# antgroup/ant-ray

Measured on NVIDIA H100. Metric: resnet50_ddp_train_images_per_sec, higher is better.
Workload: dtype bf16

## Files before the change

ant-ray_b200/csrc/inst_norm.cu:

```cuda
#include <algorithm>
#include <initializer_list>
#include <type_traits>

#include "norm_act.cuh"
#include "norm_infer.cuh"
#include "norm_kernels.cuh"
#include "norm_launch.h"
#include "norm_res.cuh"

namespace b200c {
namespace bn {

static int ceil_div(int a, int b) { return (a + b - 1) / b; }

static int last_pow2(unsigned n) {
  n |= (n >> 1);
  n |= (n >> 2);
  n |= (n >> 4);
  n |= (n >> 8);
  n |= (n >> 16);
  return std::max<int>(1, n - (n >> 1));
}

static void reduce_config(int reduction, int stride, dim3* block, dim3* grid) {
  int block_x = std::min(last_pow2(stride), kTileW);
  int block_y = std::min(last_pow2(ceil_div(reduction, kElemsPerThread)), kMaxBlock / block_x);
  if (block_x * block_y != kMaxBlock) block_x = std::min(last_pow2(stride), kMaxBlock / block_y);
  int grid_y = std::min(ceil_div(reduction, block_y * kElemsPerThread), kMaxHBlock);
  *block = dim3(block_x, block_y, 1);
  *grid = dim3(ceil_div(stride, block_x), grid_y < 8 ? 1 : grid_y, 1);
}

static_assert(kEwVec % kStatsVec == 0, "vec_ok covers the statistics kernel's vector width");
static bool vec_ok(int stride, const void* const* ptrs, int n) {
  if (stride % kEwVec) return false;
  for (int i = 0; i < n; i++)
    if (reinterpret_cast<uintptr_t>(ptrs[i]) % 16) return false;
  return true;
}

constexpr size_t kBlockSmem = 48 * 1024;
constexpr size_t kStatsStaticSmem = 3 * kMaxBlock * 4 + 16;
constexpr size_t kBwdStaticSmem = 2 * kMaxBlock * 4 + 16;

static size_t stats_ring_bytes(dim3 block) {
  return (size_t)kStatsStages * kParallelLoads * block.x * block.y * sizeof(BVec<kStatsVec>);
}
static_assert(kStatsStaticSmem + (size_t)kStatsStages * kParallelLoads * (kMaxBlock / kStatsVec) * sizeof(BVec<kStatsVec>) <= kBlockSmem,
              "the statistics ring fits every block");

static_assert(kBwdStaticSmem + (size_t)kBwdStagesWide * 5 * kParallelLoads * (kMaxBlock / kBwdVec) * sizeof(BVec<kBwdVec>) <= kBlockSmem &&
                  kBwdStaticSmem + (size_t)kBwdStages * 2 * kParallelLoads * (kMaxBlock / kBwdVec) * sizeof(BVec<kBwdVec>) <= kBlockSmem,
              "the backward ring fits every block: 2 stages of up to 5 operands, 3 of 2");
struct BwdReduceLaunch {
  dim3 block, grid;
  int vec;
  size_t smem;
};
static BwdReduceLaunch bwd_reduce_launch(int m, int c, GradSrc src, bool dy2, bool dual, const void* const* ptrs, int n) {
  BwdReduceLaunch l;
  reduce_config(m, c, &l.block, &l.grid);
  l.vec = 1;
  l.smem = 0;
  if (src == kGradPool || !vec_ok(c, ptrs, n)) return l;
  const int ops = bwd_ring_operands(src == kGradY, dy2, dual);
  const size_t ring = (size_t)bwd_ring_stages(ops) * ops * kParallelLoads * (l.block.x / kBwdVec) * l.block.y * sizeof(BVec<kBwdVec>);
  l.block.x /= kBwdVec;
  l.vec = kBwdVec;
  l.smem = ring;
  return l;
}

static void ew_config(int reduction, int stride, int vec, dim3* block, dim3* grid) {
  const int groups = stride / vec;
  const int bx = std::min(groups, kEwThreads);
  const int by = kEwThreads / bx;
  const int gx = ceil_div(groups, bx);
  const int gy = std::max(1, std::min(ceil_div(reduction, by), 4096 / gx));
  *block = dim3(bx, by, 1);
  *grid = dim3(gx, gy, 1);
}

constexpr int kSemaphores = kMaxChannels / kTileW;
constexpr size_t kSemaphoreBytes = (size_t)kSemaphores * 4;

size_t scratch_bytes(int stride) {
  return kSemaphoreBytes + (size_t)3 * stride * kMaxHBlock * 4 + (size_t)2 * stride * 4;
}

struct Scratch {
  int* semaphores;
  float* staging;
  float* sums;
};
static Scratch carve(void* scratch, int stride) {
  char* p = static_cast<char*>(scratch);
  Scratch s;
  s.semaphores = reinterpret_cast<int*>(p);
  s.staging = reinterpret_cast<float*>(p + kSemaphoreBytes);
  s.sums = s.staging + (size_t)3 * stride * kMaxHBlock;
  return s;
}

template <int... Cs, typename F>
static auto with_const(int key, F&& f) {
  std::common_type_t<decltype(f(std::integral_constant<int, Cs>{}))...> kernel = nullptr;
  ((key == Cs ? void(kernel = f(std::integral_constant<int, Cs>{})) : void()), ...);
  return kernel;
}

using StatsKernel = void (*)(const bf16*, StatsOut, volatile float*, int*, int, int);
using SyncStatsKernel = void (*)(const bf16*, float*, float, volatile float*, int*, int, int);
using StatsDualKernel = void (*)(const bf16*, const bf16*, StatsOut, StatsOut, volatile float*, volatile float*, int*, int, int);
using TransformKernel = void (*)(const bf16*, const bf16*, bf16*, uint8_t*, const float*, const float*, const float*, const float*,
                                 const float*, const float*, const float*, const float*, int, int);
using PoolFwdKernel = void (*)(const bf16*, bf16*, uint8_t*, const float*, const float*, const float*, const float*, PoolDims, int, int);
using BwdReduceKernel = void (*)(const bf16*, const bf16*, const bf16*, const bf16*, const uint8_t*, bf16*, const float*, const float*,
                                 float*, float*, float*, float*, volatile float*, int*, PoolDims, const bf16*, const float*, const float*,
                                 float*, float*, float*, int, int, int);
using BwdElemtKernel = void (*)(const bf16*, const bf16*, const bf16*, const uint8_t*, const bf16*, bf16*, const float*, const float*,
                                const float*, const float*, const float*, const float*, float, const bf16*, bf16*, const float*,
                                const float*, const float*, const float*, int, int);

static StatsKernel stats_kernel(int vec) {
  return with_const<1, kStatsVec>(vec, [](auto v) -> StatsKernel { return k_bn_stats<decltype(v)::value>; });
}
static StatsDualKernel stats_dual_kernel(int vec) {
  return with_const<1, kStatsVec>(vec, [](auto v) -> StatsDualKernel { return k_bn_stats_dual<decltype(v)::value>; });
}
static SyncStatsKernel sync_stats_kernel(int vec) {
  return with_const<1, kStatsVec>(vec, [](auto v) -> SyncStatsKernel { return k_bn_sync_stats<decltype(v)::value>; });
}
static TransformKernel transform_kernel(int vec, int tail) {
  return with_const<1, kEwVec>(vec, [&](auto v) {
    return with_const<kTailNone, kTailRelu, kTailAddRelu, kTailBnAddRelu>(
        tail, [](auto t) -> TransformKernel { return k_bn_transform<decltype(v)::value, (Tail) decltype(t)::value>; });
  });
}
static PoolFwdKernel pool_fwd_kernel(int vec) {
  return with_const<1, kEwVec>(vec, [](auto v) -> PoolFwdKernel { return k_bn_pool_fwd<decltype(v)::value>; });
}
static BwdReduceKernel bwd_reduce_kernel(int src, bool dual) {
  if (dual)
    return with_const<kGradY, kGradBits>(src, [](auto g) -> BwdReduceKernel { return k_bn_bwd_reduce<(GradSrc) decltype(g)::value, true>; });
  return with_const<kGradY, kGradBits, kGradDy, kGradPool>(
      src, [](auto g) -> BwdReduceKernel { return k_bn_bwd_reduce<(GradSrc) decltype(g)::value, false>; });
}
static BwdElemtKernel bwd_elemt_kernel(int vec, int src, bool fct_ptr, bool dual) {
  return with_const<1, kEwVec>(vec, [&](auto v) {
    if (dual)
      return with_const<kGradY, kGradBits>(src, [](auto g) -> BwdElemtKernel {
        return k_bn_bwd_elemt<decltype(v)::value, (GradSrc) decltype(g)::value, false, true>;
      });
    return with_const<kGradMasked, kGradY, kGradBits, kGradDy>(src, [&](auto g) {
      auto kernel = [](auto p) -> BwdElemtKernel {
        return k_bn_bwd_elemt<decltype(v)::value, (GradSrc) decltype(g)::value, decltype(p)::value != 0, false>;
      };
      if constexpr (decltype(g)::value == kGradDy) return with_const<true>(fct_ptr, kernel);
      else return with_const<false, true>(fct_ptr, kernel);
    });
  });
}

template <typename P>
using InferTransformKernel = void (*)(const bf16*, const bf16*, bf16*, const P*, const P*, const P*, const P*, float, const P*, const P*,
                                      const P*, const P*, float, int, int);
template <typename P>
using InferPoolKernel = void (*)(const bf16*, bf16*, const P*, const P*, const P*, const P*, float, PoolDims, int, int);

template <typename P>
static InferTransformKernel<P> infer_transform_kernel(int vec, int tail) {
  return with_const<1, kEwVec>(vec, [&](auto v) {
    return with_const<kTailRelu, kTailAddRelu, kTailBnAddRelu>(tail, [](auto t) -> InferTransformKernel<P> {
      return bn_infer::k_infer_transform<decltype(v)::value, (Tail) decltype(t)::value, P>;
    });
  });
}
template <typename P>
static InferPoolKernel<P> infer_pool_kernel(int vec) {
  return with_const<1, kEwVec>(vec, [](auto v) -> InferPoolKernel<P> { return bn_infer::k_infer_pool<decltype(v)::value, P>; });
}

using bn_act::Act;
using ActTransformKernel = void (*)(const bf16*, bf16*, const float*, const float*, const float*, const float*, int, int);
using ActBwdReduceKernel = void (*)(const bf16*, const bf16*, const float*, const float*, const float*, const float*, float*, float*,
// ... 37 lines not shown
}
static ResBwdReduceKernel res_bwd_reduce_kernel() { return bn_res::k_res_bwd_reduce; }
template <typename P>
static ResInferKernel<P> res_infer_kernel(int vec, bool add) {
  return with_const<1, kEwVec>(vec, [&](auto v) -> ResInferKernel<P> {
    return add ? bn_res::k_res_infer<decltype(v)::value, bn_res::kResAdd, P> : bn_res::k_res_infer<decltype(v)::value, bn_res::kResPlain, P>;
  });
}

cudaError_t load_kernels() {
  cudaFuncAttributes attr;
  cudaError_t e = cudaSuccess;
  auto load = [&](auto kernel) { if (kernel && e == cudaSuccess) e = cudaFuncGetAttributes(&attr, kernel); };
  load(&k_bn_sync_merge);
  load(res_bwd_reduce_kernel());
  for (int src = 0; src < kGradSrcs; src++) {
    load(bwd_reduce_kernel(src, false));
    load(bwd_reduce_kernel(src, true));
  }
  for (int vec : {1, kStatsVec, kEwVec}) {
    load(stats_kernel(vec));
    load(stats_dual_kernel(vec));
    load(sync_stats_kernel(vec));
    load(pool_fwd_kernel(vec));
    for (int tail = 0; tail < kTails; tail++) load(transform_kernel(vec, tail));
    for (int src = 0; src < kGradSrcs; src++)
      for (bool fct_ptr : {false, true})
        for (bool dual : {false, true}) load(bwd_elemt_kernel(vec, src, fct_ptr, dual));
    load(infer_pool_kernel<float>(vec));
    load(infer_pool_kernel<bf16>(vec));
    for (int tail = 0; tail < kTails; tail++) {
      load(infer_transform_kernel<float>(vec, tail));
      load(infer_transform_kernel<bf16>(vec, tail));
    }
    for (int act : {bn_act::kActRelu6, bn_act::kActSilu, bn_act::kActHardswish}) {
      if (vec == 1) load(act_bwd_reduce_kernel(act));
      load(act_transform_kernel(vec, act));
      load(act_infer_kernel<float>(vec, act));
      load(act_infer_kernel<bf16>(vec, act));
    }
    for (bool b : {false, true}) {
      load(res_transform_kernel(vec, b));
      load(res_infer_kernel<float>(vec, b));
      load(res_infer_kernel<bf16>(vec, b));
    }
  }
  return e;
}

constexpr cudaError_t kNoKernel = cudaErrorInvalidDeviceFunction;

static cudaError_t launch_stats(const FwdArgs& a, float* sync_row, cudaStream_t st) {
  Scratch s = carve(a.scratch, a.c);
  dim3 block, grid;
  reduce_config(a.m, a.c, &block, &grid);
  const int vec = vec_ok(a.c, &a.x, 1) ? kStatsVec : 1;
  block.x /= vec;
  const size_t smem = vec == kStatsVec ? stats_ring_bytes(block) : 0;
  const bf16* x = static_cast<const bf16*>(a.x);
  if (sync_row) {
    const SyncStatsKernel k = sync_stats_kernel(vec);
    if (!k) return kNoKernel;
    k<<<grid, block, smem, st>>>(x, sync_row, a.eps, s.staging, s.semaphores, a.m, a.c);
  } else {
    const StatsKernel k = stats_kernel(vec);
    if (!k) return kNoKernel;
    StatsOut o{a.save_mean, a.save_invstd, a.running_mean, a.running_var, a.num_batches_tracked, a.momentum,
               (float)((double)a.m / (double)(a.m - 1)), a.eps};
    k<<<grid, block, smem, st>>>(x, o, s.staging, s.semaphores, a.m, a.c);
  }
  return cudaGetLastError();
}

static cudaError_t launch_transform(const FwdArgs& a, cudaStream_t st) {
  const void* ptrs[3] = {a.x, a.y, a.identity ? a.identity : a.x};
  const int vec = vec_ok(a.c, ptrs, 3) ? kEwVec : 1;
  dim3 block, grid;
  ew_config(a.m, a.c, vec, &block, &grid);
  const TransformKernel k = transform_kernel(vec, !a.relu ? kTailNone : a.identity ? kTailAddRelu : kTailRelu);
  if (!k) return kNoKernel;
  k<<<grid, block, 0, st>>>(static_cast<const bf16*>(a.x), static_cast<const bf16*>(a.identity), static_cast<bf16*>(a.y),
                            static_cast<uint8_t*>(a.mask), a.save_mean, a.save_invstd, a.weight, a.bias, nullptr, nullptr, nullptr,
                            nullptr, a.m, a.c);
  return cudaGetLastError();
}

static PoolDims pool_dims(int h, int w) { return PoolDims{h, w, (h - 1) / 2 + 1, (w - 1) / 2 + 1}; }

static cudaError_t launch_pool_fwd(const FwdArgs& a, cudaStream_t st) {
  const PoolDims d = pool_dims(a.pool_h, a.pool_w);
  const int pooled_rows = a.m / (a.pool_h * a.pool_w) * d.oh * d.ow;
  const void* ptrs[3] = {a.x, a.y, a.argmax};
  const int vec = vec_ok(a.c, ptrs, 3) ? kEwVec : 1;
  dim3 block, grid;
  ew_config(pooled_rows, a.c, vec, &block, &grid);
  const PoolFwdKernel k = pool_fwd_kernel(vec);
  if (!k) return kNoKernel;
  k<<<grid, block, 0, st>>>(static_cast<const bf16*>(a.x), static_cast<bf16*>(a.y), static_cast<uint8_t*>(a.argmax), a.save_mean,
                            a.save_invstd, a.weight, a.bias, d, pooled_rows, a.c);
  return cudaGetLastError();
}

cudaError_t forward(const FwdArgs& a, cudaStream_t st) {
  const cudaError_t e = launch_stats(a, nullptr, st);
  if (e != cudaSuccess) return e;
  return a.pool_h ? launch_pool_fwd(a, st) : launch_transform(a, st);
}

static GradSrc grad_src(const BwdArgs& a, bool reduced) {
  if (!a.relu) return kGradDy;
  if (reduced && a.dy_masked) return kGradMasked;
  if (a.pool_h) return kGradPool;
  return a.mask ? kGradBits : kGradY;
}

static cudaError_t launch_bwd_reduce(const BwdArgs& a, cudaStream_t st) {
  Scratch s = carve(a.scratch, a.c);
  const GradSrc src = grad_src(a, false);
  const void* ptrs[5] = {a.x, a.dy, a.dy2 ? a.dy2 : a.dy, src == kGradY ? a.y : a.dy, a.dy_masked ? a.dy_masked : a.dy};
  const BwdReduceLaunch l = bwd_reduce_launch(a.m, a.c, src, a.dy2 != nullptr, false, ptrs, 5);
  const BwdReduceKernel k = bwd_reduce_kernel(src, false);
  if (!k) return kNoKernel;
  const void* mask = src == kGradPool ? a.argmax : a.mask;
  k<<<l.grid, l.block, l.smem, st>>>(static_cast<const bf16*>(a.x), static_cast<const bf16*>(a.dy), static_cast<const bf16*>(a.dy2),
                            static_cast<const bf16*>(a.y), static_cast<const uint8_t*>(mask), static_cast<bf16*>(a.dy_masked),
                            a.save_mean, a.save_invstd, s.sums, s.sums + a.c, a.grad_weight, a.grad_bias, s.staging, s.semaphores,
                            pool_dims(a.pool_h, a.pool_w), nullptr, nullptr, nullptr, nullptr, nullptr, nullptr, a.m, a.c, l.vec);
  return cudaGetLastError();
}

static cudaError_t launch_bwd_elemt(const BwdArgs& a, cudaStream_t st) {
  Scratch s = carve(a.scratch, a.c);
  const GradSrc src = grad_src(a, true);
  const void* g = src == kGradMasked ? a.dy_masked : a.dy;
  const void* ptrs[5] = {a.x, a.dx, g, a.dy2 && src != kGradMasked ? a.dy2 : a.dy, a.y};
  const int vec = vec_ok(a.c, ptrs, src == kGradY ? 5 : 4) ? kEwVec : 1;
  dim3 block, grid;
  ew_config(a.m, a.c, vec, &block, &grid);
  const BwdElemtKernel k = bwd_elemt_kernel(vec, src, a.norm_fct != nullptr, false);
  if (!k) return kNoKernel;
  k<<<grid, block, 0, st>>>(static_cast<const bf16*>(g), static_cast<const bf16*>(a.dy2), static_cast<const bf16*>(a.y),
                            static_cast<const uint8_t*>(a.mask), static_cast<const bf16*>(a.x), static_cast<bf16*>(a.dx), a.save_mean,
                            a.save_invstd, a.weight, s.sums, s.sums + a.c, a.norm_fct, (float)(1.0 / a.m), nullptr, nullptr, nullptr,
                            nullptr, nullptr, nullptr, a.m, a.c);
  return cudaGetLastError();
}

cudaError_t backward(const BwdArgs& a, cudaStream_t st) {
  const cudaError_t e = launch_bwd_reduce(a, st);
  return e == cudaSuccess ? launch_bwd_elemt(a, st) : e;
}

static size_t dual_extra_offset(int c) { return (scratch_bytes(c) + 15) / 16 * 16; }
size_t dual_scratch_bytes(int c) { return dual_extra_offset(c) + (size_t)3 * c * kMaxHBlock * 4 + (size_t)c * 4; }
static float* dual_staging(void* scratch, int c) { return reinterpret_cast<float*>(static_cast<char*>(scratch) + dual_extra_offset(c)); }
static float* dual_sum_xmu2(void* scratch, int c) { return dual_staging(scratch, c) + (size_t)3 * c * kMaxHBlock; }

cudaError_t forward_dual(const FwdArgs& a, const FwdArgs& b, cudaStream_t st) {
  Scratch s = carve(a.scratch, a.c);
  dim3 block, grid;
  reduce_config(a.m, a.c, &block, &grid);
  const void* xs[2] = {a.x, b.x};
  const int svec = vec_ok(a.c, xs, 2) ? kStatsVec : 1;
  block.x /= svec;
  grid.z = 2;
  const size_t smem = svec == kStatsVec ? stats_ring_bytes(block) : 0;
  const StatsDualKernel ks = stats_dual_kernel(svec);
  if (!ks) return kNoKernel;
  StatsOut oa{a.save_mean, a.save_invstd, a.running_mean, a.running_var, a.num_batches_tracked, a.momentum,
              (float)((double)a.m / (double)(a.m - 1)), a.eps};
  StatsOut ob{b.save_mean, b.save_invstd, b.running_mean, b.running_var, b.num_batches_tracked, b.momentum,
              (float)((double)b.m / (double)(b.m - 1)), b.eps};
  ks<<<grid, block, smem, st>>>(static_cast<const bf16*>(a.x), static_cast<const bf16*>(b.x), oa, ob, s.staging,
                             dual_staging(a.scratch, a.c), s.semaphores, a.m, a.c);
  cudaError_t e = cudaGetLastError();
  if (e != cudaSuccess) return e;
  const void* ptrs[3] = {a.x, a.y, b.x};
  const int vec = vec_ok(a.c, ptrs, 3) ? kEwVec : 1;
  ew_config(a.m, a.c, vec, &block, &grid);
  const TransformKernel kt = transform_kernel(vec, kTailBnAddRelu);
  if (!kt) return kNoKernel;
  kt<<<grid, block, 0, st>>>(static_cast<const bf16*>(a.x), static_cast<const bf16*>(b.x), static_cast<bf16*>(a.y),
                             static_cast<uint8_t*>(a.mask), a.save_mean, a.save_invstd, a.weight, a.bias, b.save_mean, b.save_invstd,
                             b.weight, b.bias, a.m, a.c);
  return cudaGetLastError();
}

cudaError_t backward_dual(const BwdArgs& a, const BwdArgs& b, cudaStream_t st) {
  Scratch s = carve(a.scratch, a.c);
  float* sum2 = dual_sum_xmu2(a.scratch, a.c);
  const GradSrc src = a.mask ? kGradBits : kGradY;
  const void* rptrs[5] = {a.x, a.dy, a.dy2 ? a.dy2 : a.dy, src == kGradY ? a.y : a.dy, b.x};
  const BwdReduceLaunch l = bwd_reduce_launch(a.m, a.c, src, a.dy2 != nullptr, true, rptrs, 5);
  const BwdReduceKernel kr = bwd_reduce_kernel(src, true);
  if (!kr) return kNoKernel;
  kr<<<l.grid, l.block, l.smem, st>>>(static_cast<const bf16*>(a.x), static_cast<const bf16*>(a.dy), static_cast<const bf16*>(a.dy2),
                             static_cast<const bf16*>(a.y), static_cast<const uint8_t*>(a.mask), nullptr, a.save_mean, a.save_invstd,
                             s.sums, s.sums + a.c, a.grad_weight, a.grad_bias, s.staging, s.semaphores, pool_dims(0, 0),
                             static_cast<const bf16*>(b.x), b.save_mean, b.save_invstd, sum2, b.grad_weight, b.grad_bias, a.m, a.c, l.vec);
  cudaError_t e = cudaGetLastError();
  if (e != cudaSuccess) return e;
  const void* ptrs[7] = {a.x, a.dx, a.dy, a.dy2 ? a.dy2 : a.dy, b.x, b.dx, a.y};
  const int vec = vec_ok(a.c, ptrs, src == kGradY ? 7 : 6) ? kEwVec : 1;
  dim3 block, grid;
  ew_config(a.m, a.c, vec, &block, &grid);
  const BwdElemtKernel ke = bwd_elemt_kernel(vec, src, false, true);
  if (!ke) return kNoKernel;
  ke<<<grid, block, 0, st>>>(static_cast<const bf16*>(a.dy), static_cast<const bf16*>(a.dy2), static_cast<const bf16*>(a.y),
                             static_cast<const uint8_t*>(a.mask), static_cast<const bf16*>(a.x), static_cast<bf16*>(a.dx), a.save_mean,
                             a.save_invstd, a.weight, s.sums, s.sums + a.c, nullptr, (float)(1.0 / a.m), static_cast<const bf16*>(b.x),
                             static_cast<bf16*>(b.dx), b.save_mean, b.save_invstd, b.weight, sum2, a.m, a.c);
  return cudaGetLastError();
}

template <typename P>
static cudaError_t launch_infer(const InferArgs& a, cudaStream_t st) {
  auto p = [](const void* q) { return static_cast<const P*>(q); };
  const bf16* x = static_cast<const bf16*>(a.x);
  bf16* y = static_cast<bf16*>(a.y);
  const InferParams& b = a.bn;
  dim3 block, grid;
  if (a.pool_h) {
    const PoolDims d = pool_dims(a.pool_h, a.pool_w);
    const int pooled_rows = a.m / (a.pool_h * a.pool_w) * d.oh * d.ow;
    const void* ptrs[2] = {a.x, a.y};
    const int vec = vec_ok(a.c, ptrs, 2) ? kEwVec : 1;
    ew_config(pooled_rows, a.c, vec, &block, &grid);
    const InferPoolKernel<P> k = infer_pool_kernel<P>(vec);
    if (!k) return kNoKernel;
    k<<<grid, block, 0, st>>>(x, y, p(b.running_mean), p(b.running_var), p(b.weight), p(b.bias), b.eps, d, pooled_rows, a.c);
    return cudaGetLastError();
// ... 167 lines not shown
```

ant-ray_b200/csrc/norm_kernels.cuh:

```cuda
#pragma once
#include <cuda_bf16.h>
#include <cuda_runtime.h>
#include <stdint.h>

#include <type_traits>

namespace b200c {
namespace bn {

constexpr int kMaxBlock = 512;
constexpr int kParallelLoads = 4;
constexpr int kElemsPerThread = 16;
constexpr int kTileW = 32;
constexpr int kMaxHBlock = 128;
constexpr int kStatsVec = 4;
constexpr int kBwdVec = 4;
constexpr int kStatsStages = 4;
constexpr unsigned kBwdStages = 3;
constexpr unsigned kBwdStagesWide = 2;
__host__ __device__ constexpr unsigned bwd_ring_stages(int ops) { return ops >= 3 ? kBwdStagesWide : kBwdStages; }
__host__ __device__ constexpr int bwd_ring_operands(bool y, bool dy2, bool dual) { return 2 + dy2 + y + dual; }
constexpr int kEwThreads = 256;
constexpr int kEwVec = 8;

typedef __nv_bfloat16 bf16;

template <int V>
struct alignas(2 * V) BVec {
  bf16 v[V];
};

__device__ __forceinline__ unsigned char* ring_smem() {
  extern __shared__ __align__(16) unsigned char bn_ring[];
  return bn_ring;
}
template <int BYTES>
__device__ __forceinline__ void cp_async(void* smem, const void* gmem) {
  asm volatile("cp.async.ca.shared.global [%0], [%1], %2;\n" ::"r"((unsigned)__cvta_generic_to_shared(smem)), "l"(gmem), "n"(BYTES)
               : "memory");
}
__device__ __forceinline__ void cp_async_commit() { asm volatile("cp.async.commit_group;\n" ::: "memory"); }
template <int N>
__device__ __forceinline__ void cp_async_wait() { asm volatile("cp.async.wait_group %0;\n" ::"n"(N) : "memory"); }


template <bool FUSE_NEW>
__device__ __forceinline__ void welford_merge_element(int& count, float& mean, float& m2n, const int& count_new,
                                                      const float& mean_new, const float& m2n_new) {
  float factor = float(1.0) / ::max(1, (count + count_new));
  float delta0 = mean - mean_new;
  const float c = count, c_new = count_new;
  mean = __fmul_rn(FUSE_NEW ? __fmaf_rn(mean_new, c_new, __fmul_rn(mean, c)) : __fmaf_rn(mean, c, __fmul_rn(mean_new, c_new)),
                   factor);
  m2n = __fadd_rn(m2n, __fmaf_rn(__fmul_rn(__fmul_rn(__fmul_rn(delta0, delta0), c_new), c), factor, m2n_new));
  count += count_new;
}

template <int V>
__device__ __forceinline__ void welford_merge_block_vertical(int (&count)[V], float (&mean)[V], float (&m2n)[V],
                                                             int* shmem_count, float* shmem_mean, float* shmem_m2n) {
  const int block_x = blockDim.x * V;
  auto address_base = threadIdx.x * V + threadIdx.y * block_x;
#pragma unroll
  for (int offset = blockDim.y / 2; offset > 0; offset >>= 1) {
    if (threadIdx.y < offset * 2) {
#pragma unroll
      for (int k = 0; k < V; k++) {
        shmem_mean[address_base + k] = mean[k];
        shmem_m2n[address_base + k] = m2n[k];
        shmem_count[address_base + k] = count[k];
      }
    }
    __syncthreads();
    if (threadIdx.y < offset && threadIdx.y + offset < blockDim.y) {
      auto address = address_base + offset * block_x;
#pragma unroll
      for (int k = 0; k < V; k++) {
        auto count_new = shmem_count[address + k];
        auto mean_new = shmem_mean[address + k];
        auto m2n_new = shmem_m2n[address + k];
        welford_merge_element<false>(count[k], mean[k], m2n[k], count_new, mean_new, m2n_new);
      }
    }
  }
}

template <int V>
__device__ __forceinline__ void merge_block_vertical_backward(float (&sum_dy)[V], float (&sum_dy_xmu)[V], float* shmem_sum_dy,
                                                              float* shmem_sum_dy_xmu) {
  const int block_x = blockDim.x * V;
  auto address_base = threadIdx.x * V + threadIdx.y * block_x;
#pragma unroll
  for (int offset = blockDim.y / 2; offset > 0; offset >>= 1) {
    if (threadIdx.y < offset * 2) {
#pragma unroll
      for (int k = 0; k < V; k++) {
        shmem_sum_dy[address_base + k] = sum_dy[k];
        shmem_sum_dy_xmu[address_base + k] = sum_dy_xmu[k];
      }
    }
    __syncthreads();
    if (threadIdx.y < offset && threadIdx.y + offset < blockDim.y) {
      auto address = address_base + offset * block_x;
#pragma unroll
      for (int k = 0; k < V; k++) {
        sum_dy[k] += shmem_sum_dy[address + k];
        sum_dy_xmu[k] += shmem_sum_dy_xmu[address + k];
      }
    }
  }
}

__device__ __forceinline__ void merge_block_vertical_backward(float& sum_dy, float& sum_dy_xmu, float* shmem_sum_dy,
                                                              float* shmem_sum_dy_xmu) {
  float a[1] = {sum_dy}, b[1] = {sum_dy_xmu};
  merge_block_vertical_backward<1>(a, b, shmem_sum_dy, shmem_sum_dy_xmu);
  sum_dy = a[0];
  sum_dy_xmu = b[0];
}

struct StatsOut {
  float* save_mean;
  float* save_invstd;
  float* running_mean;
  float* running_var;
  long long* num_batches_tracked;
  float momentum, bessel, eps;
};

__device__ __forceinline__ void finish_stats(const StatsOut& o, int c, float mean_th, float m2_th, int count_th) {
  const float mean = mean_th;
  const float var = m2_th / count_th;
  const float momentum = o.momentum;
  const float unbiased_var = var * o.bessel;
  o.save_mean[c] = mean;
  o.running_mean[c] = __fmaf_rn(mean, momentum, __fmul_rn(1 - momentum, o.running_mean[c]));
  o.running_var[c] = __fmaf_rn(unbiased_var, momentum, __fmul_rn(1 - momentum, o.running_var[c]));
  o.save_invstd[c] = rsqrtf(var + o.eps);
}

template <int V, typename Finish>
__device__ __forceinline__ void bn_stats_body(const bf16* __restrict__ input, volatile float* staging_data, int* semaphores,
                                              const int reduction_size, const int stride, Finish finish) {
  constexpr int PARALLEL_LOADS = kParallelLoads;
  float x_mean[PARALLEL_LOADS][V];
  float m_2_n[PARALLEL_LOADS][V];
  int count[PARALLEL_LOADS];
#pragma unroll
  for (int i = 0; i < PARALLEL_LOADS; i++) {
#pragma unroll
    for (int k = 0; k < V; k++) {
      x_mean[i][k] = 0.f;
      m_2_n[i][k] = 0.f;
    }
    count[i] = 0;
  }

  int inner_loop_stride = blockDim.y * gridDim.y;
  int m_offset = blockIdx.y * blockDim.y + threadIdx.y;
  int c_offset = (blockIdx.x * blockDim.x + threadIdx.x) * V;
  int loop_count = 1 + (reduction_size - 1) / (inner_loop_stride * PARALLEL_LOADS);
  const bool c_valid = c_offset < stride;

  auto update = [&](int j, const BVec<V>* xv) {
    float x_math[V];
    float x_count_inv;
    float is_valid;
    if (c_valid && m_offset < reduction_size) {
      const BVec<V> x = *xv;
#pragma unroll
      for (int k = 0; k < V; k++) x_math[k] = __bfloat162float(x.v[k]);
      count[j]++;
      x_count_inv = float(1) / count[j];
      is_valid = float(1);
    } else {
#pragma unroll
      for (int k = 0; k < V; k++) x_math[k] = float(0);
      x_count_inv = float(0);
      is_valid = float(0);
    }
    m_offset += inner_loop_stride;
#pragma unroll
    for (int k = 0; k < V; k++) {
      float delta0 = x_math[k] - x_mean[j][k];
      x_mean[j][k] = __fmaf_rn(delta0, x_count_inv, x_mean[j][k]);
      float delta1 = x_math[k] - x_mean[j][k];
      m_2_n[j][k] = __fmaf_rn(__fmul_rn(delta0, delta1), is_valid, m_2_n[j][k]);
    }
  };

  if constexpr (V == 1) {
    for (int i = 0; i < loop_count; i++) {
      BVec<V> xv[PARALLEL_LOADS];
#pragma unroll
      for (int j = 0; j < PARALLEL_LOADS; j++) {
        const int m = m_offset + j * inner_loop_stride;
        if (c_valid && m < reduction_size) xv[j] = *reinterpret_cast<const BVec<V>*>(input + ((size_t)m * stride + c_offset));
      }
#pragma unroll
      for (int j = 0; j < PARALLEL_LOADS; j++) update(j, &xv[j]);
    }
  } else {
    constexpr unsigned D = kStatsStages;
    const int threads = blockDim.x * blockDim.y;
    BVec<V>* ring = reinterpret_cast<BVec<V>*>(ring_smem()) + threadIdx.y * blockDim.x + threadIdx.x;
    const int first_row = m_offset;
    auto issue = [&](unsigned it) {
      BVec<V>* slot = ring + (it % D) * PARALLEL_LOADS * threads;
      int m = first_row + (int)it * PARALLEL_LOADS * inner_loop_stride;
#pragma unroll
      for (int j = 0; j < PARALLEL_LOADS; j++, m += inner_loop_stride)
        if (c_valid && m < reduction_size) cp_async<sizeof(BVec<V>)>(slot + j * threads, input + ((size_t)m * stride + c_offset));
      cp_async_commit();
    };
#pragma unroll
    for (unsigned it = 0; it < D - 1; it++) issue(it);
    for (unsigned i = 0; i < (unsigned)loop_count; i++) {
      issue(i + D - 1);
      cp_async_wait<D - 1>();
      const BVec<V>* slot = ring + (i % D) * PARALLEL_LOADS * threads;
#pragma unroll
      for (int j = 0; j < PARALLEL_LOADS; j++) update(j, slot + j * threads);
    }
  }
  float mean_th[V], m2_th[V];
  int count_th[V];
#pragma unroll
  for (int k = 0; k < V; k++) {
    count_th[k] = count[0];
    mean_th[k] = x_mean[0][k];
    m2_th[k] = m_2_n[0][k];
#pragma unroll
    for (int j = 1; j < PARALLEL_LOADS; j++) welford_merge_element<true>(count_th[k], mean_th[k], m2_th[k], count[j], x_mean[j][k], m_2_n[j][k]);
  }

  __shared__ float shmem_mean[kMaxBlock];
  __shared__ float shmem_m2n[kMaxBlock];
  __shared__ int shmem_count[kMaxBlock];
  welford_merge_block_vertical<V>(count_th, mean_th, m2_th, shmem_count, shmem_mean, shmem_m2n);

  if (gridDim.y > 1) {
    volatile float* staging_mean = staging_data;
    volatile float* staging_m2n = &staging_data[stride * gridDim.y];
    volatile int* staging_count = reinterpret_cast<volatile int*>(&staging_m2n[stride * gridDim.y]);
    int address_base = c_offset + blockIdx.y * stride;
    if (threadIdx.y == 0 && c_valid) {
#pragma unroll
      for (int k = 0; k < V; k++) {
        staging_mean[address_base + k] = mean_th[k];
        staging_m2n[address_base + k] = m2_th[k];
        staging_count[address_base + k] = count_th[k];
      }
    }
    __threadfence();
    __syncthreads();
    __shared__ bool is_last_block_done;
    if (threadIdx.x == 0 && threadIdx.y == 0) {
      int old = atomicAdd(&semaphores[blockIdx.x], 1);
      is_last_block_done = (old == (gridDim.y - 1));
      if (is_last_block_done) semaphores[blockIdx.x] = 0;
    }
    __syncthreads();
    if (is_last_block_done) {
#pragma unroll
      for (int k = 0; k < V; k++) {
        count_th[k] = 0;
        mean_th[k] = float(0.0);
        m2_th[k] = float(0.0);
      }
      for (int y = threadIdx.y; y < gridDim.y; y += blockDim.y) {
        address_base = c_offset + y * stride;
#pragma unroll
        for (int k = 0; k < V; k++) {
          int count_new = c_valid ? staging_count[address_base + k] : 0;
          float mean_new = c_valid ? staging_mean[address_base + k] : float(0.0);
          float m2n_new = c_valid ? staging_m2n[address_base + k] : float(0.0);
          welford_merge_element<false>(count_th[k], mean_th[k], m2_th[k], count_new, mean_new, m2n_new);
        }
      }
      welford_merge_block_vertical<V>(count_th, mean_th, m2_th, shmem_count, shmem_mean, shmem_m2n);
      if (threadIdx.y == 0 && c_valid)
#pragma unroll
        for (int k = 0; k < V; k++) finish(c_offset + k, mean_th[k], m2_th[k], count_th[k]);
    }
  } else {
    if (blockIdx.y == 0 && threadIdx.y == 0 && c_valid)
#pragma unroll
      for (int k = 0; k < V; k++) finish(c_offset + k, mean_th[k], m2_th[k], count_th[k]);
  }
}

template <int V>
__global__ void __launch_bounds__(kMaxBlock / V) k_bn_stats(const bf16* __restrict__ input, StatsOut o, volatile float* staging_data,
                                                            int* semaphores, const int reduction_size, const int stride) {
  if (o.num_batches_tracked && blockIdx.x == 0 && blockIdx.y == 0 && threadIdx.x == 0 && threadIdx.y == 0)
    *o.num_batches_tracked += 1;
  bn_stats_body<V>(input, staging_data, semaphores, reduction_size, stride,
                   [&](int c, float mean, float m2n, int count) { finish_stats(o, c, mean, m2n, count); });
}

template <int V>
__global__ void __launch_bounds__(kMaxBlock / V) k_bn_stats_dual(const bf16* __restrict__ input0, const bf16* __restrict__ input1,
                                                                 StatsOut o0, StatsOut o1, volatile float* staging0,
                                                                 volatile float* staging1, int* semaphores, const int reduction_size,
                                                                 const int stride) {
  const bool z = blockIdx.z != 0;
  const StatsOut o{z ? o1.save_mean : o0.save_mean, z ? o1.save_invstd : o0.save_invstd, z ? o1.running_mean : o0.running_mean,
                   z ? o1.running_var : o0.running_var, z ? o1.num_batches_tracked : o0.num_batches_tracked,
                   z ? o1.momentum : o0.momentum, z ? o1.bessel : o0.bessel, z ? o1.eps : o0.eps};
  if (o.num_batches_tracked && blockIdx.x == 0 && blockIdx.y == 0 && threadIdx.x == 0 && threadIdx.y == 0)
    *o.num_batches_tracked += 1;
  bn_stats_body<V>(z ? input1 : input0, z ? staging1 : staging0, semaphores + (z ? gridDim.x : 0), reduction_size, stride,
                   [&](int c, float mean, float m2n, int count) { finish_stats(o, c, mean, m2n, count); });
}


template <int V>
__global__ void __launch_bounds__(kMaxBlock / V) k_bn_sync_stats(const bf16* __restrict__ input, float* __restrict__ local,
                                                                 const float eps, volatile float* staging_data, int* semaphores,
                                                                 const int reduction_size, const int stride) {
  if (blockIdx.x == 0 && blockIdx.y == 0 && threadIdx.x == 0 && threadIdx.y == 0) local[2 * stride] = (float)reduction_size;
  bn_stats_body<V>(input, staging_data, semaphores, reduction_size, stride, [&](int c, float mean, float m2n, int count) {
    const float var = m2n / count;
    local[c] = mean;
    local[stride + c] = (var != 0.f || eps != 0.f) ? (float)(1.0 / sqrt((double)var + (double)eps)) : 0.f;
  });
}

__global__ void __launch_bounds__(kEwThreads) k_bn_sync_merge(const float* __restrict__ rows, const int row_stride, const int world,
                                                              float* __restrict__ save_mean, float* __restrict__ save_invstd,
                                                              float* __restrict__ norm_fct, float* __restrict__ running_mean,
                                                              float* __restrict__ running_var, long long* num_batches_tracked,
                                                              const float momentum, const float eps, const int stride) {
  const int i = blockIdx.x * blockDim.x + threadIdx.x;
  if (i == 0) {
    long long total = 0;
    for (int j = 0; j < world; j++) {
      const float count = rows[(size_t)j * row_stride + 2 * stride];
      if (count >= 1.f) total += (int)count;
    }
    *norm_fct = 1.f / (float)total;
    if (num_batches_tracked) *num_batches_tracked += 1;
  }
  if (i >= stride) return;
  float avg = 0.f, var_n = 0.f;
  int n = 0;
  for (int j = 0; j < world; j++) {
    const float* row = rows + (size_t)j * row_stride;
    const float count = row[2 * stride];
    if (!(count >= 1.f)) continue;
    const float m = row[i];
    float v = __fdiv_rn(1.f, row[stride + i]);
    v = __fmaf_rn(v, v, -eps);
    const float nf = (float)n;
    const float factor = __fdiv_rn(1.f, __fadd_rn(nf, count));
    const float d = __fsub_rn(avg, m);
    const float t = __fmul_rn(__fmul_rn(__fmul_rn(__fmul_rn(d, d), nf), count), factor);
    var_n = __fadd_rn(var_n, __fmaf_rn(v, count, t));
    avg = __fmaf_rn(__fmul_rn(nf, factor), avg, __fmul_rn(__fmul_rn(count, factor), m));
    n = (int)__fadd_rn(nf, count);
  }
  save_mean[i] = avg;
  save_invstd[i] = __fdiv_rn(1.f, __fsqrt_rn(__fadd_rn(__fdiv_rn(var_n, (float)n), eps)));
  running_mean[i] = __fmaf_rn(avg, momentum, __fmul_rn(1 - momentum, running_mean[i]));
  const float unbiased_var = __fdiv_rn(var_n, (float)(n - 1));
  running_var[i] = __fmaf_rn(unbiased_var, momentum, __fmul_rn(1 - momentum, running_var[i]));
}

enum Tail { kTailNone, kTailRelu, kTailAddRelu, kTailBnAddRelu };
constexpr int kTails = 4;

template <int V, Tail TAIL>
__global__ void __launch_bounds__(kEwThreads) k_bn_transform(const bf16* __restrict__ input, const bf16* __restrict__ identity,
                                                             bf16* __restrict__ out, uint8_t* __restrict__ mask,
                                                             const float* __restrict__ mean, const float* __restrict__ inv_std,
// ... 445 lines not shown
```

Measured before the change: 5627.

## Split BN stats channel groups across four lanes when the grid underfills the GPU

Adds a four-lane mode to the BN statistics kernels. Each channel vector's parallel loads are spread over four threads with their own cp.async ring of depth 8, and the partial Welford results are merged with shuffles before the block-level reduction. The mode is picked at launch from a cached per-device occupancy query, when the grid fits in one wave, and an environment variable can force either mode. It aims to raise memory parallelism for small-grid stats launches, at the cost of more threads per block, extra shuffle merges, changed launch bounds that may affect register allocation, and a getenv call on every launch.

```diff
diff --git a/ant-ray_b200/csrc/inst_norm.cu b/ant-ray_b200/csrc/inst_norm.cu
--- a/ant-ray_b200/csrc/inst_norm.cu
+++ b/ant-ray_b200/csrc/inst_norm.cu
@@ -1,5 +1,7 @@
 #include <algorithm>
+#include <cstdlib>
 #include <initializer_list>
+#include <mutex>
 #include <type_traits>
 
 #include "norm_act.cuh"
@@ -43,11 +45,14 @@
 constexpr size_t kStatsStaticSmem = 3 * kMaxBlock * 4 + 16;
 constexpr size_t kBwdStaticSmem = 2 * kMaxBlock * 4 + 16;
 
-static size_t stats_ring_bytes(dim3 block) {
-  return (size_t)kStatsStages * kParallelLoads * block.x * block.y * sizeof(BVec<kStatsVec>);
-}
-static_assert(kStatsStaticSmem + (size_t)kStatsStages * kParallelLoads * (kMaxBlock / kStatsVec) * sizeof(BVec<kStatsVec>) <= kBlockSmem,
-              "the statistics ring fits every block");
+static size_t stats_ring_bytes(int threads, int lanes) {
+  return (size_t)stats_ring_stages(lanes) * (kParallelLoads / lanes) * threads * sizeof(BVec<kStatsVec>);
+}
+constexpr size_t stats_ring_bound(int lanes) {
+  return kStatsStaticSmem + (size_t)stats_ring_stages(lanes) * (kParallelLoads / lanes) * lanes * (kMaxBlock / kStatsVec) * sizeof(BVec<kStatsVec>);
+}
+static_assert(stats_ring_bound(1) <= kBlockSmem, "the statistics ring fits every block with one lane");
+static_assert(stats_ring_bound(kStatsMaxLanes) <= kBlockSmem, "the statistics ring fits every block with four lanes");
 
 static_assert(kBwdStaticSmem + (size_t)kBwdStagesWide * 5 * kParallelLoads * (kMaxBlock / kBwdVec) * sizeof(BVec<kBwdVec>) <= kBlockSmem &&
                   kBwdStaticSmem + (size_t)kBwdStages * 2 * kParallelLoads * (kMaxBlock / kBwdVec) * sizeof(BVec<kBwdVec>) <= kBlockSmem,
@@ -109,9 +114,9 @@
   return kernel;
 }
 
-using StatsKernel = void (*)(const bf16*, StatsOut, volatile float*, int*, int, int);
-using SyncStatsKernel = void (*)(const bf16*, float*, float, volatile float*, int*, int, int);
-using StatsDualKernel = void (*)(const bf16*, const bf16*, StatsOut, StatsOut, volatile float*, volatile float*, int*, int, int);
+using StatsKernel = void (*)(const bf16*, StatsOut, volatile float*, int*, int, int, int);
+using SyncStatsKernel = void (*)(const bf16*, float*, float, volatile float*, int*, int, int, int);
+using StatsDualKernel = void (*)(const bf16*, const bf16*, StatsOut, StatsOut, volatile float*, volatile float*, int*, int, int, int);
 using TransformKernel = void (*)(const bf16*, const bf16*, bf16*, uint8_t*, const float*, const float*, const float*, const float*,
                                  const float*, const float*, const float*, const float*, int, int);
 using PoolFwdKernel = void (*)(const bf16*, bf16*, uint8_t*, const float*, const float*, const float*, const float*, PoolDims, int, int);
@@ -131,6 +136,67 @@
 static SyncStatsKernel sync_stats_kernel(int vec) {
   return with_const<1, kStatsVec>(vec, [](auto v) -> SyncStatsKernel { return k_bn_sync_stats<decltype(v)::value>; });
 }
+
+enum StatsKind { kStatsLocal, kStatsDual, kStatsSync, kStatsKinds };
+struct StatsResidency {
+  bool known = false;
+  int sms = 0;
+  int lanes_blocks_per_sm[kStatsKinds] = {};
+};
+static const void* stats_kernel_ptr(StatsKind kind) {
+  return kind == kStatsDual ? (const void*)stats_dual_kernel(kStatsVec)
+         : kind == kStatsSync ? (const void*)sync_stats_kernel(kStatsVec) : (const void*)stats_kernel(kStatsVec);
+}
+constexpr int kMaxDevices = 64;
+static StatsResidency stats_residency() {
+  static std::mutex mu;
+  static StatsResidency per_device[kMaxDevices];
+  int dev = 0;
+  if (cudaGetDevice(&dev) != cudaSuccess || dev < 0 || dev >= kMaxDevices) {
+    cudaGetLastError();
+    return StatsResidency{};
+  }
+  std::lock_guard<std::mutex> lock(mu);
+  StatsResidency& r = per_device[dev];
+  if (!r.known) {
+    const int threads = kStatsMaxLanes * (kMaxBlock / kStatsVec);
+    cudaDeviceGetAttribute(&r.sms, cudaDevAttrMultiProcessorCount, dev);
+    for (int kind = 0; kind < kStatsKinds; kind++)
+      cudaOccupancyMaxActiveBlocksPerMultiprocessor(&r.lanes_blocks_per_sm[kind], stats_kernel_ptr((StatsKind)kind), threads,
+                                                    stats_ring_bytes(threads, kStatsMaxLanes));
+    cudaGetLastError();
+    r.known = true;
+  }
+  return r;
+}
+
+struct StatsLaunch {
+  dim3 block, grid;
+  int vec, lanes;
+  size_t smem;
+};
+static StatsLaunch stats_launch(int m, int c, int planes, const void* const* xs, int n, StatsKind kind) {
+  StatsLaunch l;
+  reduce_config(m, c, &l.block, &l.grid);
+  l.grid.z = planes;
+  l.vec = vec_ok(c, xs, n) ? kStatsVec : 1;
+  l.lanes = 1;
+  l.smem = 0;
+  if (l.vec == 1) return l;
+  const char* forced = std::getenv("B200C_BN_STATS_LANES");
+  const int want = forced ? std::atoi(forced) : 0;
+  if (want == 1 || want == kStatsMaxLanes) {
+    l.lanes = want;
+  } else {
+    const StatsResidency r = stats_residency();
+    const long long blocks = (long long)l.grid.x * l.grid.y * l.grid.z;
+    if (blocks <= (long long)r.lanes_blocks_per_sm[kind] * r.sms) l.lanes = kStatsMaxLanes;
+  }
+  l.block.x = l.block.x / kStatsVec * l.lanes;
+  l.smem = stats_ring_bytes(l.block.x * l.block.y, l.lanes);
+  return l;
+}
+
 static TransformKernel transform_kernel(int vec, int tail) {
   return with_const<1, kEwVec>(vec, [&](auto v) {
     return with_const<kTailNone, kTailRelu, kTailAddRelu, kTailBnAddRelu>(
@@ -274,22 +340,18 @@
 
 static cudaError_t launch_stats(const FwdArgs& a, float* sync_row, cudaStream_t st) {
   Scratch s = carve(a.scratch, a.c);
-  dim3 block, grid;
-  reduce_config(a.m, a.c, &block, &grid);
-  const int vec = vec_ok(a.c, &a.x, 1) ? kStatsVec : 1;
-  block.x /= vec;
-  const size_t smem = vec == kStatsVec ? stats_ring_bytes(block) : 0;
+  const StatsLaunch l = stats_launch(a.m, a.c, 1, &a.x, 1, sync_row ? kStatsSync : kStatsLocal);
   const bf16* x = static_cast<const bf16*>(a.x);
   if (sync_row) {
-    const SyncStatsKernel k = sync_stats_kernel(vec);
+    const SyncStatsKernel k = sync_stats_kernel(l.vec);
     if (!k) return kNoKernel;
-    k<<<grid, block, smem, st>>>(x, sync_row, a.eps, s.staging, s.semaphores, a.m, a.c);
+    k<<<l.grid, l.block, l.smem, st>>>(x, sync_row, a.eps, s.staging, s.semaphores, a.m, a.c, l.lanes);
   } else {
-    const StatsKernel k = stats_kernel(vec);
+    const StatsKernel k = stats_kernel(l.vec);
     if (!k) return kNoKernel;
     StatsOut o{a.save_mean, a.save_invstd, a.running_mean, a.running_var, a.num_batches_tracked, a.momentum,
                (float)((double)a.m / (double)(a.m - 1)), a.eps};
-    k<<<grid, block, smem, st>>>(x, o, s.staging, s.semaphores, a.m, a.c);
+    k<<<l.grid, l.block, l.smem, st>>>(x, o, s.staging, s.semaphores, a.m, a.c, l.lanes);
   }
   return cudaGetLastError();
 }
@@ -380,25 +442,21 @@
 
 cudaError_t forward_dual(const FwdArgs& a, const FwdArgs& b, cudaStream_t st) {
   Scratch s = carve(a.scratch, a.c);
-  dim3 block, grid;
-  reduce_config(a.m, a.c, &block, &grid);
   const void* xs[2] = {a.x, b.x};
-  const int svec = vec_ok(a.c, xs, 2) ? kStatsVec : 1;
-  block.x /= svec;
-  grid.z = 2;
-  const size_t smem = svec == kStatsVec ? stats_ring_bytes(block) : 0;
-  const StatsDualKernel ks = stats_dual_kernel(svec);
+  const StatsLaunch l = stats_launch(a.m, a.c, 2, xs, 2, kStatsDual);
+  const StatsDualKernel ks = stats_dual_kernel(l.vec);
   if (!ks) return kNoKernel;
   StatsOut oa{a.save_mean, a.save_invstd, a.running_mean, a.running_var, a.num_batches_tracked, a.momentum,
               (float)((double)a.m / (double)(a.m - 1)), a.eps};
   StatsOut ob{b.save_mean, b.save_invstd, b.running_mean, b.running_var, b.num_batches_tracked, b.momentum,
               (float)((double)b.m / (double)(b.m - 1)), b.eps};
-  ks<<<grid, block, smem, st>>>(static_cast<const bf16*>(a.x), static_cast<const bf16*>(b.x), oa, ob, s.staging,
-                             dual_staging(a.scratch, a.c), s.semaphores, a.m, a.c);
+  ks<<<l.grid, l.block, l.smem, st>>>(static_cast<const bf16*>(a.x), static_cast<const bf16*>(b.x), oa, ob, s.staging,
+                                     dual_staging(a.scratch, a.c), s.semaphores, a.m, a.c, l.lanes);
   cudaError_t e = cudaGetLastError();
   if (e != cudaSuccess) return e;
   const void* ptrs[3] = {a.x, a.y, b.x};
   const int vec = vec_ok(a.c, ptrs, 3) ? kEwVec : 1;
+  dim3 block, grid;
   ew_config(a.m, a.c, vec, &block, &grid);
   const TransformKernel kt = transform_kernel(vec, kTailBnAddRelu);
   if (!kt) return kNoKernel;
diff --git a/ant-ray_b200/csrc/norm_kernels.cuh b/ant-ray_b200/csrc/norm_kernels.cuh
--- a/ant-ray_b200/csrc/norm_kernels.cuh
+++ b/ant-ray_b200/csrc/norm_kernels.cuh
@@ -15,7 +15,10 @@
 constexpr int kMaxHBlock = 128;
 constexpr int kStatsVec = 4;
 constexpr int kBwdVec = 4;
+constexpr int kStatsMaxLanes = 4;
 constexpr int kStatsStages = 4;
+constexpr int kStatsStagesLanes = 8;
+__host__ __device__ constexpr int stats_ring_stages(int lanes) { return lanes == 1 ? kStatsStages : kStatsStagesLanes; }
 constexpr unsigned kBwdStages = 3;
 constexpr unsigned kBwdStagesWide = 2;
 __host__ __device__ constexpr unsigned bwd_ring_stages(int ops) { return ops >= 3 ? kBwdStagesWide : kBwdStages; }
@@ -58,12 +61,13 @@
 
 template <int V>
 __device__ __forceinline__ void welford_merge_block_vertical(int (&count)[V], float (&mean)[V], float (&m2n)[V],
-                                                             int* shmem_count, float* shmem_mean, float* shmem_m2n) {
-  const int block_x = blockDim.x * V;
-  auto address_base = threadIdx.x * V + threadIdx.y * block_x;
+                                                             int* shmem_count, float* shmem_mean, float* shmem_m2n, const int tx,
+                                                             const int bdx, const bool owner) {
+  const int block_x = bdx * V;
+  auto address_base = tx * V + threadIdx.y * block_x;
 #pragma unroll
   for (int offset = blockDim.y / 2; offset > 0; offset >>= 1) {
-    if (threadIdx.y < offset * 2) {
+    if (owner && threadIdx.y < offset * 2) {
 #pragma unroll
       for (int k = 0; k < V; k++) {
         shmem_mean[address_base + k] = mean[k];
@@ -72,7 +76,7 @@
       }
     }
     __syncthreads();
-    if (threadIdx.y < offset && threadIdx.y + offset < blockDim.y) {
+    if (owner && threadIdx.y < offset && threadIdx.y + offset < blockDim.y) {
       auto address = address_base + offset * block_x;
 #pragma unroll
       for (int k = 0; k < V; k++) {
@@ -140,8 +144,9 @@
 }
 
 template <int V, typename Finish>
-__device__ __forceinline__ void bn_stats_body(const bf16* __restrict__ input, volatile float* staging_data, int* semaphores,
-                                              const int reduction_size, const int stride, Finish finish) {
+__device__ __forceinline__ void bn_stats_one_lane(const bf16* __restrict__ input, volatile float* staging_data, int* semaphores,
+                                                  const int reduction_size, const int stride, float* shmem_mean, float* shmem_m2n,
+                                                  int* shmem_count, bool& is_last_block_done, Finish finish) {
   constexpr int PARALLEL_LOADS = kParallelLoads;
   float x_mean[PARALLEL_LOADS][V];
   float m_2_n[PARALLEL_LOADS][V];
@@ -234,10 +239,7 @@
     for (int j = 1; j < PARALLEL_LOADS; j++) welford_merge_element<true>(count_th[k], mean_th[k], m2_th[k], count[j], x_mean[j][k], m_2_n[j][k]);
   }
 
-  __shared__ float shmem_mean[kMaxBlock];
-  __shared__ float shmem_m2n[kMaxBlock];
-  __shared__ int shmem_count[kMaxBlock];
-  welford_merge_block_vertical<V>(count_th, mean_th, m2_th, shmem_count, shmem_mean, shmem_m2n);
+  welford_merge_block_vertical<V>(count_th, mean_th, m2_th, shmem_count, shmem_mean, shmem_m2n, threadIdx.x, blockDim.x, true);
 
   if (gridDim.y > 1) {
     volatile float* staging_mean = staging_data;
@@ -254,7 +256,6 @@
     }
     __threadfence();
     __syncthreads();
-    __shared__ bool is_last_block_done;
     if (threadIdx.x == 0 && threadIdx.y == 0) {
       int old = atomicAdd(&semaphores[blockIdx.x], 1);
       is_last_block_done = (old == (gridDim.y - 1));
@@ -278,7 +279,7 @@
           welford_merge_element<false>(count_th[k], mean_th[k], m2_th[k], count_new, mean_new, m2n_new);
         }
       }
-      welford_merge_block_vertical<V>(count_th, mean_th, m2_th, shmem_count, shmem_mean, shmem_m2n);
+      welford_merge_block_vertical<V>(count_th, mean_th, m2_th, shmem_count, shmem_mean, shmem_m2n, threadIdx.x, blockDim.x, true);
       if (threadIdx.y == 0 && c_valid)
 #pragma unroll
         for (int k = 0; k < V; k++) finish(c_offset + k, mean_th[k], m2_th[k], count_th[k]);
@@ -290,37 +291,213 @@
   }
 }
 
+template <int V, typename Finish>
+__device__ __forceinline__ void bn_stats_four_lanes(const bf16* __restrict__ input, volatile float* staging_data, int* semaphores,
+                                                    const int reduction_size, const int stride, float* shmem_mean, float* shmem_m2n,
+                                                    int* shmem_count, bool& is_last_block_done, Finish finish) {
+  constexpr int PARALLEL_LOADS = kParallelLoads;
+  constexpr int L = kStatsMaxLanes;
+  constexpr int CHAINS = PARALLEL_LOADS / L;
+  float x_mean[CHAINS][V];
+  float m_2_n[CHAINS][V];
+  int count[CHAINS];
+#pragma unroll
+  for (int i = 0; i < CHAINS; i++) {
+#pragma unroll
+    for (int k = 0; k < V; k++) {
+      x_mean[i][k] = 0.f;
+      m_2_n[i][k] = 0.f;
+    }
+    count[i] = 0;
+  }
+
+  const int tx = threadIdx.x / L, bdx = blockDim.x / L;
+  const int lane = threadIdx.x % L;
+  const bool owner = lane == 0;
+  int inner_loop_stride = blockDim.y * gridDim.y;
+  int m_offset = blockIdx.y * blockDim.y + threadIdx.y;
+  int c_offset = (blockIdx.x * bdx + tx) * V;
+  int loop_count = 1 + (reduction_size - 1) / (inner_loop_stride * PARALLEL_LOADS);
+  const bool c_valid = c_offset < stride;
+
+  auto update = [&](int j, int m, const BVec<V>* xv) {
+    float x_math[V];
+    float x_count_inv;
+    float is_valid;
+    if (c_valid && m < reduction_size) {
+      const BVec<V> x = *xv;
+#pragma unroll
+      for (int k = 0; k < V; k++) x_math[k] = __bfloat162float(x.v[k]);
+      count[j]++;
+      x_count_inv = float(1) / count[j];
+      is_valid = float(1);
+    } else {
+#pragma unroll
+      for (int k = 0; k < V; k++) x_math[k] = float(0);
+      x_count_inv = float(0);
+      is_valid = float(0);
+    }
+#pragma unroll
+    for (int k = 0; k < V; k++) {
+      float delta0 = x_math[k] - x_mean[j][k];
+      x_mean[j][k] = __fmaf_rn(delta0, x_count_inv, x_mean[j][k]);
+      float delta1 = x_math[k] - x_mean[j][k];
+      m_2_n[j][k] = __fmaf_rn(__fmul_rn(delta0, delta1), is_valid, m_2_n[j][k]);
+    }
+  };
+
+  constexpr unsigned D = stats_ring_stages(L);
+  const int threads = blockDim.x * blockDim.y;
+  BVec<V>* ring = reinterpret_cast<BVec<V>*>(ring_smem()) + threadIdx.y * blockDim.x + threadIdx.x;
+  const int first_row = m_offset + lane * CHAINS * inner_loop_stride;
+  auto issue = [&](unsigned it) {
+    BVec<V>* slot = ring + (it % D) * CHAINS * threads;
+    int m = first_row + (int)it * PARALLEL_LOADS * inner_loop_stride;
+#pragma unroll
+    for (int q = 0; q < CHAINS; q++, m += inner_loop_stride)
+      if (c_valid && m < reduction_size) cp_async<sizeof(BVec<V>)>(slot + q * threads, input + ((size_t)m * stride + c_offset));
+    cp_async_commit();
+  };
+#pragma unroll
+  for (unsigned it = 0; it < D - 1; it++) issue(it);
+  for (unsigned i = 0; i < (unsigned)loop_count; i++) {
+    issue(i + D - 1);
+    cp_async_wait<D - 1>();
+    const BVec<V>* slot = ring + (i % D) * CHAINS * threads;
+    const int m = first_row + (int)i * PARALLEL_LOADS * inner_loop_stride;
+#pragma unroll
+    for (int q = 0; q < CHAINS; q++) update(q, m + q * inner_loop_stride, slot + q * threads);
+  }
+  float mean_th[V], m2_th[V];
+  int count_th[V];
+#pragma unroll
+  for (int k = 0; k < V; k++) {
+    count_th[k] = count[0];
+    mean_th[k] = x_mean[0][k];
+    m2_th[k] = m_2_n[0][k];
+#pragma unroll
+    for (int j = 1; j < CHAINS; j++) welford_merge_element<true>(count_th[k], mean_th[k], m2_th[k], count[j], x_mean[j][k], m_2_n[j][k]);
+  }
+  {
+    const unsigned warp_lane = (threadIdx.y * blockDim.x + threadIdx.x) % 32;
+    const unsigned group = ((1u << L) - 1) << (warp_lane & ~(unsigned)(L - 1));
+#pragma unroll
+    for (int j = CHAINS; j < PARALLEL_LOADS; j++) {
+      const int src = j / CHAINS, q = j % CHAINS;
+      const int count_new = __shfl_sync(group, count[q], src, L);
+#pragma unroll
+      for (int k = 0; k < V; k++) {
+        const float mean_new = __shfl_sync(group, x_mean[q][k], src, L);
+        const float m2n_new = __shfl_sync(group, m_2_n[q][k], src, L);
+        welford_merge_element<true>(count_th[k], mean_th[k], m2_th[k], count_new, mean_new, m2n_new);
+      }
+    }
+  }
+
+  welford_merge_block_vertical<V>(count_th, mean_th, m2_th, shmem_count, shmem_mean, shmem_m2n, tx, bdx, owner);
+
+  if (gridDim.y > 1) {
+    volatile float* staging_mean = staging_data;
+    volatile float* staging_m2n = &staging_data[stride * gridDim.y];
+    volatile int* staging_count = reinterpret_cast<volatile int*>(&staging_m2n[stride * gridDim.y]);
+    int address_base = c_offset + blockIdx.y * stride;
+    if (owner && threadIdx.y == 0 && c_valid) {
+#pragma unroll
+      for (int k = 0; k < V; k++) {
+        staging_mean[address_base + k] = mean_th[k];
+        staging_m2n[address_base + k] = m2_th[k];
+        staging_count[address_base + k] = count_th[k];
+      }
+    }
+    __threadfence();
+    __syncthreads();
+    if (threadIdx.x == 0 && threadIdx.y == 0) {
+      int old = atomicAdd(&semaphores[blockIdx.x], 1);
+      is_last_block_done = (old == (gridDim.y - 1));
+      if (is_last_block_done) semaphores[blockIdx.x] = 0;
+    }
+    __syncthreads();
+    if (is_last_block_done) {
+#pragma unroll
+      for (int k = 0; k < V; k++) {
+        count_th[k] = 0;
+        mean_th[k] = float(0.0);
+        m2_th[k] = float(0.0);
+      }
+      if (owner) {
+        for (int y = threadIdx.y; y < gridDim.y; y += blockDim.y) {
+          address_base = c_offset + y * stride;
+#pragma unroll
+          for (int k = 0; k < V; k++) {
+            int count_new = c_valid ? staging_count[address_base + k] : 0;
+            float mean_new = c_valid ? staging_mean[address_base + k] : float(0.0);
+            float m2n_new = c_valid ? staging_m2n[address_base + k] : float(0.0);
+            welford_merge_element<false>(count_th[k], mean_th[k], m2_th[k], count_new, mean_new, m2n_new);
+          }
+        }
+      }
+      welford_merge_block_vertical<V>(count_th, mean_th, m2_th, shmem_count, shmem_mean, shmem_m2n, tx, bdx, owner);
+      if (owner && threadIdx.y == 0 && c_valid)
+#pragma unroll
+        for (int k = 0; k < V; k++) finish(c_offset + k, mean_th[k], m2_th[k], count_th[k]);
+    }
+  } else {
+    if (owner && blockIdx.y == 0 && threadIdx.y == 0 && c_valid)
+#pragma unroll
+      for (int k = 0; k < V; k++) finish(c_offset + k, mean_th[k], m2_th[k], count_th[k]);
+  }
+}
+
+template <int V, typename Finish>
+__device__ __forceinline__ void bn_stats_body(const bf16* __restrict__ input, volatile float* staging_data, int* semaphores,
+                                              const int reduction_size, const int stride, const int lanes, Finish finish) {
+  __shared__ float shmem_mean[kMaxBlock];
+  __shared__ float shmem_m2n[kMaxBlock];
+  __shared__ int shmem_count[kMaxBlock];
+  __shared__ bool is_last_block_done;
+  if constexpr (V != 1) {
+    if (lanes == kStatsMaxLanes) {
+      bn_stats_four_lanes<V>(input, staging_data, semaphores, reduction_size, stride, shmem_mean, shmem_m2n, shmem_count,
+                             is_last_block_done, finish);
+      return;
+    }
+  }
+  bn_stats_one_lane<V>(input, staging_data, semaphores, reduction_size, stride, shmem_mean, shmem_m2n, shmem_count,
+                       is_last_block_done, finish);
+}
+
 template <int V>
-__global__ void __launch_bounds__(kMaxBlock / V) k_bn_stats(const bf16* __restrict__ input, StatsOut o, volatile float* staging_data,
-                                                            int* semaphores, const int reduction_size, const int stride) {
+__global__ void __launch_bounds__(kMaxBlock, V == 1 ? 0 : 2) k_bn_stats(const bf16* __restrict__ input, StatsOut o, volatile float* staging_data,
+                                                            int* semaphores, const int reduction_size, const int stride,
+                                                            const int lanes) {
   if (o.num_batches_tracked && blockIdx.x == 0 && blockIdx.y == 0 && threadIdx.x == 0 && threadIdx.y == 0)
     *o.num_batches_tracked += 1;
-  bn_stats_body<V>(input, staging_data, semaphores, reduction_size, stride,
+  bn_stats_body<V>(input, staging_data, semaphores, reduction_size, stride, lanes,
                    [&](int c, float mean, float m2n, int count) { finish_stats(o, c, mean, m2n, count); });
 }
 
 template <int V>
-__global__ void __launch_bounds__(kMaxBlock / V) k_bn_stats_dual(const bf16* __restrict__ input0, const bf16* __restrict__ input1,
+__global__ void __launch_bounds__(kMaxBlock, V == 1 ? 0 : 2) k_bn_stats_dual(const bf16* __restrict__ input0, const bf16* __restrict__ input1,
                                                                  StatsOut o0, StatsOut o1, volatile float* staging0,
                                                                  volatile float* staging1, int* semaphores, const int reduction_size,
-                                                                 const int stride) {
+                                                                 const int stride, const int lanes) {
   const bool z = blockIdx.z != 0;
   const StatsOut o{z ? o1.save_mean : o0.save_mean, z ? o1.save_invstd : o0.save_invstd, z ? o1.running_mean : o0.running_mean,
                    z ? o1.running_var : o0.running_var, z ? o1.num_batches_tracked : o0.num_batches_tracked,
                    z ? o1.momentum : o0.momentum, z ? o1.bessel : o0.bessel, z ? o1.eps : o0.eps};
   if (o.num_batches_tracked && blockIdx.x == 0 && blockIdx.y == 0 && threadIdx.x == 0 && threadIdx.y == 0)
     *o.num_batches_tracked += 1;
-  bn_stats_body<V>(z ? input1 : input0, z ? staging1 : staging0, semaphores + (z ? gridDim.x : 0), reduction_size, stride,
+  bn_stats_body<V>(z ? input1 : input0, z ? staging1 : staging0, semaphores + (z ? gridDim.x : 0), reduction_size, stride, lanes,
                    [&](int c, float mean, float m2n, int count) { finish_stats(o, c, mean, m2n, count); });
 }
 
 
 template <int V>
-__global__ void __launch_bounds__(kMaxBlock / V) k_bn_sync_stats(const bf16* __restrict__ input, float* __restrict__ local,
+__global__ void __launch_bounds__(kMaxBlock, V == 1 ? 0 : 2) k_bn_sync_stats(const bf16* __restrict__ input, float* __restrict__ local,
                                                                  const float eps, volatile float* staging_data, int* semaphores,
-                                                                 const int reduction_size, const int stride) {
+                                                                 const int reduction_size, const int stride, const int lanes) {
   if (blockIdx.x == 0 && blockIdx.y == 0 && threadIdx.x == 0 && threadIdx.y == 0) local[2 * stride] = (float)reduction_size;
-  bn_stats_body<V>(input, staging_data, semaphores, reduction_size, stride, [&](int c, float mean, float m2n, int count) {
+  bn_stats_body<V>(input, staging_data, semaphores, reduction_size, stride, lanes, [&](int c, float mean, float m2n, int count) {
     const float var = m2n / count;
     local[c] = mean;
     local[stride + c] = (var != 0.f || eps != 0.f) ? (float)(1.0 / sqrt((double)var + (double)eps)) : 0.f;
```

New measurement: 5668, median of 6. No clear change (+0.7%).
